# rwl/blu

Hardware: AMD Instinct MI355X
Metric: factorize nnz/s + achieved HBM GB/s, 100k x 100k 10-nnz/col basis (higher is better)
Workload: dtype f64

## Files before the change

### blu_amd/csrc/k_chain.h

```cpp
#pragma once
#include "blu_dev.h"

#define CH_SB 32
#define CH_NB 8
#define CH_CS (CH_SB * CH_NB)
#define CH_CE 4096
#define CH_W 2048
#define CH_FAR 320
#define CH_HAS 0x10000
#define CH_HT 16
#define CH_SEL_FAR (-1)
#define CH_SEL_PREV (-2)

struct __attribute__((aligned(16))) ChRecA {
    int n, eb, w, k;
};
struct __attribute__((aligned(16))) ChRecB {
    double diag, own;
};
struct __attribute__((aligned(16))) ChOpsV {
    double val, xv;
};
struct ChainLds {
    ChOpsV ev[CH_CE];
    int sel[CH_CE];
    double xwin[CH_W];
    ChRecA ra[CH_CS];
    ChRecB rb[CH_CS];
    double rinit[CH_CS];
    long long s_b[CH_CS];
    volatile int blk_ready[CH_NB];
    volatile int eb_tag[CH_HT];
    volatile int eb_val[CH_HT];
    volatile int chain_done;
    volatile int chain_eb;
    volatile int abort;
};

struct ChMeta {
    long long b;
    int len;
    int w;
    double diag, own;
};
struct ChEnt {
    int pos;
    int gidx;
    double val;
};

#define CH_WAIT(L, cond, code)                                         \
    do {                                                            \
        int it_ = 0;                                                \
        while (!(cond)) {                                           \
            if ((L)->abort || ++it_ > (1 << 24)) {                  \
                if (!(L)->abort) (L)->abort = (code);               \
                break;                                              \
            }                                                       \
            __builtin_amdgcn_s_sleep(1);                            \
        }                                                           \
    } while (0)

#ifdef BLU_EMU_BUILD
__device__ __forceinline__ void ch_lds_fence() {}
__device__ __forceinline__ void ch_vm_drain() {}
#else
__device__ __forceinline__ void ch_lds_fence() { asm volatile("s_waitcnt lgkmcnt(0)" ::: "memory"); }
__device__ __forceinline__ void ch_vm_drain() { asm volatile("s_waitcnt vmcnt(0)" ::: "memory"); }
#endif
__device__ __forceinline__ double ch_load_final(gdouble_p p)
{
    const long long b = __hip_atomic_load((GPTR(const long long))p, __ATOMIC_RELAXED, __HIP_MEMORY_SCOPE_AGENT);
    return __longlong_as_double(b);
}

template <bool INIT_OWN, bool SUB, class A>
__device__ __forceinline__ void ch_stage_block(const A &ad, ChainLds *L, int b, int k0, int dir, int nsteps, gdouble_p out)
{
    const int lane = lane_id();
    const int s0 = b * CH_SB;
    const int ns = nsteps - s0 < CH_SB ? nsteps - s0 : CH_SB;
    const int k = k0 + dir * (s0 + (lane < ns ? lane : 0));
    ChMeta M = ad.meta(k);
    if (M.len < 0) M.len = 0;
    const bool mine = lane < ns;
    const int st = (mine && M.len <= 64) ? M.len : 0;
    const int incl = wave_incl_scan_i(st);
    const int off = incl - st;
    const int cnt = __builtin_amdgcn_readlane(incl, 63);
    int base = 0;
    if (b > 0) {
        CH_WAIT(L, L->eb_tag[b & (CH_HT - 1)] == b, 1);
        base = L->eb_val[b & (CH_HT - 1)];
    }
    if (lane == 0) {
        L->eb_val[(b + 1) & (CH_HT - 1)] = base + cnt;
        ch_lds_fence();
        L->eb_tag[(b + 1) & (CH_HT - 1)] = b + 1;
    }
    CH_WAIT(L, L->chain_done >= b - CH_NB + 1 && base + cnt - L->chain_eb <= CH_CE, 2);
    asm volatile("" ::: "memory");
    if (L->abort) return;
    const int slot0 = s0 & (CH_CS - 1);
    if (mine) {
        const int sl = slot0 + lane;
        ChRecA a;
        a.n = M.len <= 64 ? (M.len > 0 ? (M.len | CH_HAS) : 0) : -1;
        a.eb = base + off;
        a.w = M.w;
        a.k = k;
        L->ra[sl] = a;
        ChRecB bq;
        bq.diag = M.diag;
        bq.own = M.own;
        L->rb[sl] = bq;
        L->rinit[sl] = INIT_OWN ? M.own : 0.0;
        L->s_b[sl] = M.b;
    }
    ch_lds_fence();
    for (int f0 = 0; f0 < cnt; f0 += 256) {
        int tt[4], ee[4];
        ChEnt E[4];
        bool ok[4], far[4];
        double xo[4];
#pragma unroll
        for (int u = 0; u < 4; u++) {
            const int f = f0 + u * 64 + lane;
            ok[u] = f < cnt;
            int lo = 0, hi = ns - 1;
            const int target = base + (ok[u] ? f : 0);
#pragma unroll
            for (int it = 0; it < 5; it++) {
                const int mid = (lo + hi + 1) >> 1;
                const bool ge = (L->ra[slot0 + mid].eb <= target) && (mid <= hi);
                lo = ge ? mid : lo;
                hi = ge ? hi : mid - 1;
            }
            tt[u] = lo;
            ee[u] = target - L->ra[slot0 + lo].eb;
        }
#pragma unroll
        for (int u = 0; u < 4; u++) {
            E[u].pos = 0;
            E[u].gidx = 0;
            E[u].val = 0.0;
            if (ok[u]) E[u] = ad.ent(L->ra[slot0 + tt[u]].k, L->s_b[slot0 + tt[u]], ee[u]);
        }
#pragma unroll
        for (int u = 0; u < 4; u++) {
            const int kk = L->ra[slot0 + tt[u]].k;
            const int d = (kk - E[u].pos) * dir;
            far[u] = ok[u] && d >= CH_FAR;
            xo[u] = 0.0;
            if (far[u]) xo[u] = ch_load_final(out + E[u].gidx);
        }
#pragma unroll
        for (int u = 0; u < 4; u++) {
            if (ok[u]) {
                const int kk = L->ra[slot0 + tt[u]].k;
                const int r = (base + f0 + u * 64 + lane) & (CH_CE - 1);
                ChOpsV ov;
                ov.val = E[u].val;
                ov.xv = xo[u];
                L->ev[r] = ov;
                L->sel[r] = far[u] ? CH_SEL_FAR : (E[u].pos == kk - dir ? CH_SEL_PREV : (E[u].pos & (CH_W - 1)));
            }
        }
    }
    ch_lds_fence();
    if (mine && M.len > 0 && M.len <= 64) {
        const int sl = slot0 + lane;
        const int eb = base + off;
        double acc = INIT_OWN ? M.own : 0.0;
        int p = 0;
        while (p < M.len && L->sel[(eb + p) & (CH_CE - 1)] == CH_SEL_FAR) {
            const ChOpsV ov = L->ev[(eb + p) & (CH_CE - 1)];
            const double term = __dmul_rn(ov.xv, ov.val);
            acc = SUB ? __dsub_rn(acc, term) : __dadd_rn(acc, term);
            p++;
        }
        if (p > 0) {
            L->ra[sl].n = (M.len - p) | CH_HAS;
            L->ra[sl].eb = eb + p;
            L->rinit[sl] = acc;
        }
    }
    ch_lds_fence();
    if (lane == 0) L->blk_ready[b & (CH_NB - 1)] = b + 1;
}

struct ChRec {
    int n, eb, w, k;
    double diag, own, init;
};
struct ChOps {
    double val, xv;
    int sel;
};
__device__ __forceinline__ ChRec ch_read_rec(ChainLds *L, int s)
{
    const int sl = s & (CH_CS - 1);
    const ChRecA a = L->ra[sl];
    const ChRecB b = L->rb[sl];
    ChRec R;
    R.n = a.n;
    R.eb = a.eb;
    R.w = a.w;
    R.k = a.k;
    R.diag = b.diag;
    R.own = b.own;
    R.init = L->rinit[sl];
    return R;
}
__device__ __forceinline__ ChOps ch_read_ops(ChainLds *L, const ChRec &R)
{
    ChOps E;
    E.val = 0.0;
    E.xv = 0.0;
    E.sel = CH_SEL_FAR;
    if (lane_id() < (R.n & (CH_HAS - 1)) && R.n > 0) {
        const int r = (R.eb + lane_id()) & (CH_CE - 1);
        const ChOpsV v = L->ev[r];
        E.val = v.val;
        E.xv = v.xv;
        E.sel = L->sel[r];
    }
    return E;
}
template <bool SUB>
__device__ __forceinline__ double ch_accumulate(double acc, double prod, int n)
{
    const unsigned lo = (unsigned)__double_as_longlong(prod), hi = (unsigned)(__double_as_longlong(prod) >> 32);
#define CH_TERM(T)                                                                                              \
    {                                                                                                           \
        const unsigned a_ = __builtin_amdgcn_readlane(lo, (T)), b_ = __builtin_amdgcn_readlane(hi, (T));        \
        const double term_ = __longlong_as_double((long long)(((unsigned long long)b_ << 32) | a_));            \
        acc = SUB ? __dsub_rn(acc, term_) : __dadd_rn(acc, term_);                                              \
    }
    int t = 0;
    for (; t + 4 <= n; t += 4) {
        CH_TERM(t)
        CH_TERM(t + 1)
        CH_TERM(t + 2)
        CH_TERM(t + 3)
    }
    for (; t < n; t++) CH_TERM(t)
#undef CH_TERM
    return acc;
}

template <bool SUB>
__device__ __forceinline__ double ch_accumulate_rows(double acc, double prod, int n)
{
    const double sg = SUB ? -1.0 : 1.0;
#ifdef BLU_EMU_BUILD
#define CH_D(T) acc = fma(__shfl(prod, (lane_id() & ~15) + T), sg, acc);
#define CH_D0 CH_D(0)
#else
#define CH_D(T) asm volatile("v_fmac_f64_dpp %0, %1, %2 row_newbcast:" #T " row_mask:0xf bank_mask:0xf" : "+v"(acc) : "v"(prod), "v"(sg));
#define CH_D0 asm volatile("s_nop 4\n\tv_fmac_f64_dpp %0, %1, %2 row_newbcast:0 row_mask:0xf bank_mask:0xf" : "+v"(acc) : "v"(prod), "v"(sg));
#endif
#define CH_TAIL(A, B, C) \
    if (n > A) {         \
        CH_D(A)          \
        if (n > B) {     \
            CH_D(B)      \
            if (n > C) { \
                CH_D(C)  \
            }            \
        }                \
    }
    if (n >= 4) {
        CH_D0 CH_D(1) CH_D(2) CH_D(3)
        if (n >= 8) {
            CH_D(4) CH_D(5) CH_D(6) CH_D(7)
            if (n >= 12) {
                CH_D(8) CH_D(9) CH_D(10) CH_D(11)
                if (n >= 16) {
                    CH_D(12) CH_D(13) CH_D(14) CH_D(15)
                } else {
                    CH_TAIL(12, 13, 14)
                }
            } else {
                CH_TAIL(8, 9, 10)
            }
        } else {
            CH_TAIL(4, 5, 6)
        }
    } else if (n > 0) {
        CH_D0
        CH_TAIL(1, 2, 3)
    }
#undef CH_TAIL
#undef CH_D0
#undef CH_D
    return acc;
}

template <bool INIT_OWN, bool SUB, class A, class F>
__device__ __forceinline__ bool chain_sweep(const A &ad, ChainLds *L, int k0, int dir, int nsteps, gdouble_p out, F f)
{
    const int w = wave_id(), nw = num_waves(), lane = lane_id();
    const int nblk = (nsteps + CH_SB - 1) / CH_SB;
    if (threadIdx.x < CH_NB) L->blk_ready[threadIdx.x] = 0;
    if (threadIdx.x < CH_HT) L->eb_tag[threadIdx.x] = -1;
    if (threadIdx.x == 0) {
        L->chain_done = 0;
        L->chain_eb = 0;
        L->abort = 0;
    }
    __syncthreads();
    if (w > 0) {
        for (int b = w - 1; b < nblk && !L->abort; b += nw - 1) ch_stage_block<INIT_OWN, SUB>(ad, L, b, k0, dir, nsteps, out);
    } else if (nsteps > 0) {
#ifdef BLU_PROFILE
        long long t_wait = 0, t_drain = 0;
        const long long t_begin = (long long)__builtin_amdgcn_s_memtime();
#endif
        const auto wait_block = [&](int b) {
            if (b < nblk) {
                CH_WAIT(L, L->blk_ready[b & (CH_NB - 1)] == b + 1, 3);
                asm volatile("" ::: "memory");
            }
        };
        const int last = nsteps - 1;
        const auto rl_d = [](double x, int t) {
            const int lo = __builtin_amdgcn_readlane(__double2loint(x), t), hi = __builtin_amdgcn_readlane(__double2hiint(x), t);
            return __hiloint2double(hi, lo);
        };
        const auto read_ops = [&](int eb, int nf) {
            ChOps E;
            E.val = 0.0;
            E.xv = 0.0;
            E.sel = CH_SEL_FAR;
            const int n = nf < 0 ? 0 : (nf & (CH_HAS - 1));
            const int li = n <= 16 ? (lane & 15) : lane;
            if (li < n) {
                const int r = (eb + li) & (CH_CE - 1);
                const ChOpsV v = L->ev[r];
                E.val = v.val;
                E.xv = v.xv;
                E.sel = L->sel[r];
            }
            return E;
        };
        wait_block(0);
        ChRec BR;
        ChOps E1, E2;
        double xw1 = 0.0, vprev = 0.0;
        for (int b = 0; b < nblk && !L->abort; b++) {
#ifdef BLU_PROFILE
            const long long tw0 = (long long)__builtin_amdgcn_s_memtime();
#endif
            wait_block(b + 1);
#ifdef BLU_PROFILE
            t_wait += (long long)__builtin_amdgcn_s_memtime() - tw0;
#endif
            const int bs = b * CH_SB;
            {
                const int sl = bs + lane;
                BR = ch_read_rec(L, sl < last ? sl : last);
            }
            if (b == 0) {
                E1 = read_ops(__builtin_amdgcn_readlane(BR.eb, 0), __builtin_amdgcn_readlane(BR.n, 0));
                xw1 = E1.sel >= 0 ? L->xwin[E1.sel] : 0.0;
                E2 = read_ops(__builtin_amdgcn_readlane(BR.eb, 1), __builtin_amdgcn_readlane(BR.n, 1));
            }
            const int ns = (bs + CH_SB < nsteps ? CH_SB : nsteps - bs);
            for (int t = 0; t < ns; t++) {
                const double xw2 = E2.sel >= 0 ? L->xwin[E2.sel] : 0.0;
                const ChOps E3 = read_ops(__builtin_amdgcn_readlane(BR.eb, t + 2), __builtin_amdgcn_readlane(BR.n, t + 2));
                const int nf = __builtin_amdgcn_readlane(BR.n, t), k1 = __builtin_amdgcn_readlane(BR.k, t), w1 = __builtin_amdgcn_readlane(BR.w, t);
                const double own1 = rl_d(BR.own, t), diag1 = rl_d(BR.diag, t);
                const int n1 = nf < 0 ? -1 : (nf & (CH_HAS - 1));
                double acc = rl_d(BR.init, t);
                if (n1 > 0) {
                    const double x = E1.sel == CH_SEL_PREV ? vprev : (E1.sel >= 0 ? xw1 : E1.xv);
                    if (n1 <= 16) acc = ch_accumulate_rows<SUB>(acc, (lane & 15) < n1 ? __dmul_rn(x, E1.val) : 0.0, n1);
                    else acc = ch_accumulate<SUB>(acc, lane < n1 ? __dmul_rn(x, E1.val) : 0.0, n1);
                } else if (n1 < 0) {
                    const ChMeta M = ad.meta(k1);
                    for (int o = 0; o < M.len; o += 64) {
                        ChEnt E;
                        E.pos = 0;
                        E.gidx = 0;
                        E.val = 0.0;
                        const int nn = M.len - o < 64 ? M.len - o : 64;
                        if (lane < nn) E = ad.ent(k1, M.b, o + lane);
                        acc = ch_accumulate<SUB>(acc, lane < nn ? __dmul_rn(out[E.gidx], E.val) : 0.0, nn);
                    }
                }
                const double v = f(k1, nf != 0, acc, own1, diag1);
                if (lane == 0) {
                    L->xwin[k1 & (CH_W - 1)] = v;
                    out[w1] = v;
                }
                vprev = v;
                E1 = E2;
                xw1 = xw2;
                E2 = E3;
            }
#ifdef BLU_PROFILE
            const long long td0 = (long long)__builtin_amdgcn_s_memtime();
#endif
            ch_vm_drain();
#ifdef BLU_PROFILE
            t_drain += (long long)__builtin_amdgcn_s_memtime() - td0;
#endif
            ch_lds_fence();
            const int eb_next = __builtin_amdgcn_readlane(BR.eb, CH_SB);
            if (lane == 0 && bs + CH_SB < nsteps) {
                L->chain_eb = eb_next;
                L->chain_done = b + 1;
            }
        }
        ch_vm_drain();
#ifdef BLU_PROFILE
        if (lane == 0)
            printf("chain sweep (block %d): %d steps, %.0f cycles/step, waiting for blocks %.0f, draining stores %.0f\n", (int)blockIdx.x, nsteps,
                   (double)((long long)__builtin_amdgcn_s_memtime() - t_begin) / nsteps, (double)t_wait / nsteps, (double)t_drain / nsteps);
#endif
    }
    __syncthreads();
    return L->abort == 0;
}
```

### blu_amd/csrc/k_chain.hip

```cpp
#include "blu_dev.h"
#include "k_chain.h"

struct RowsWs {
    int *lt_ptr, *lt_idx;
    double *lt_val;
    int *lt_cur;
    int *ur_len;
    int *ur_pos;
    double *ur_val;
};

template <bool DESC>
__device__ __forceinline__ void insertion_sort_ik(int *key, double *val, int b, int e)
{
    for (int p = b + 1; p < e; p++) {
        const int k = key[p];
        const double v = val[p];
        int q = p - 1;
        while (q >= b && (DESC ? key[q] < k : key[q] > k)) {
            key[q + 1] = key[q];
            val[q + 1] = val[q];
            q--;
        }
        key[q + 1] = k;
        val[q + 1] = v;
    }
}
template <bool DESC>
__device__ void wave_sort_segment_ik(int *key, double *val, int b, int e, int *lk, double *lv)
{
    const int lane = lane_id();
    const int n = e - b;
    WAVE_LOCKSTEP();
    for (int t = lane; t < n; t += 64) {
        lk[t] = key[b + t];
        lv[t] = val[b + t];
    }
    __builtin_amdgcn_fence(__ATOMIC_SEQ_CST, "workgroup");
    for (int t = lane; t < n; t += 64) {
        const int k = lk[t];
        int r = 0;
        for (int u = 0; u < n; u++) r += DESC ? (lk[u] > k) : (lk[u] < k);
        key[b + r] = k;
        val[b + r] = lv[t];
    }
}

template <class Scope>
__device__ __forceinline__ void rows_body(const DevG &D, const RowsWs &R, Scope &sc, int *lds_k, double *lds_v)
{
    Scalars *S = D.s;
    const int tid = sc.tid(), nt = sc.nt();
    const int m = D.m;
    if (S->status != ST_DONE) return;
    const int rank = S->rank;
    const int lend = D.lbeg[rank];
    for (int i = tid; i < m; i += nt) R.lt_cur[i] = 0;
    if (sc.leader()) *sc.ctr(0) = *sc.ctr(1) = 0;
    sc.sync();
    for (int p = tid; p < lend; p += nt) atomicAdd(&R.lt_cur[D.lidx[p]], 1);
    sc.sync();
    int base = 0;
    for (int c0 = 0; c0 < m; c0 += nt) {
        const int i = c0 + tid;
        const int c = i < m ? R.lt_cur[i] : 0;
        int tot;
        const int ex = sc.excl_scan(c, &tot);
        if (i < m) {
            R.lt_ptr[i] = base + ex;
            R.lt_cur[i] = base + ex;
        }
        base += tot;
    }
    if (sc.leader()) R.lt_ptr[m] = base;
    sc.sync();
    for (int k = tid; k < rank; k += nt)
        for (int p = D.lbeg[k]; p < D.lbeg[k + 1]; p++) {
            const int q = atomicAdd(&R.lt_cur[D.lidx[p]], 1);
            R.lt_idx[q] = k;
            R.lt_val[q] = D.lval[p];
        }
    sc.sync();
    for (int i = tid; i < m; i += nt) {
        const int b = R.lt_ptr[i], e = R.lt_ptr[i + 1];
        if (e - b > 24 && e - b <= WSORT_MAX) D.iw2[atomicAdd(sc.ctr(0), 1)] = i;
        else insertion_sort_ik<false>(R.lt_idx, R.lt_val, b, e);
    }
    for (int k = tid; k < m; k += nt) {
        int n = 0;
        if (k < rank) {
            const int b = D.ubeg[k], e = D.ubeg[k + 1];
            for (int p = b; p < e; p++) {
                const int c = D.qinv[D.uidx[p]];
                if (c < rank) {
                    R.ur_pos[b + n] = c;
                    R.ur_val[b + n] = D.uval[p];
                    n++;
                }
            }
            if (n > 24 && n <= WSORT_MAX) D.iw1[atomicAdd(sc.ctr(1), 1)] = k;
            else insertion_sort_ik<true>(R.ur_pos, R.ur_val, b, b + n);
        }
        R.ur_len[k] = n;
    }
    sc.sync();
    {
        const int nl = __hip_atomic_load(sc.ctr(0), __ATOMIC_RELAXED, __HIP_MEMORY_SCOPE_AGENT);
        const int nu = __hip_atomic_load(sc.ctr(1), __ATOMIC_RELAXED, __HIP_MEMORY_SCOPE_AGENT);
#ifdef BLU_STATS_DEBUG
        if (sc.leader()) printf("k_rows_grid: medium L rows %d, medium U rows %d, rank %d, m %d\n", nl, nu, rank, m);
#endif
        for (int r = sc.wid(); r < nl + nu; r += sc.nw()) {
            if (r < nl) {
                const int i = D.iw2[r];
                wave_sort_segment_ik<false>(R.lt_idx, R.lt_val, R.lt_ptr[i], R.lt_ptr[i + 1], &lds_k[wave_id() * WSORT_MAX],
                                            &lds_v[wave_id() * WSORT_MAX]);
            } else {
                const int k = D.iw1[r - nl];
                wave_sort_segment_ik<true>(R.ur_pos, R.ur_val, D.ubeg[k], D.ubeg[k] + R.ur_len[k], &lds_k[wave_id() * WSORT_MAX],
                                           &lds_v[wave_id() * WSORT_MAX]);
            }
        }
    }
    sc.sync();
    for (int p = tid; p < lend; p += nt) R.lt_idx[p] = D.prow[R.lt_idx[p]];
}
__global__ void __launch_bounds__(1024) k_rows_grid(DevLU *Ds, GridWs *gw, RowsWs R)
{
    __shared__ int sh[40];
    __shared__ long long shl[20];
    __shared__ int lds_k[16 * WSORT_MAX];
    __shared__ double lds_v[16 * WSORT_MAX];
    const DevG D(Ds[0]);
    GridScope sc{sh, shl, gw, 0};
    rows_body(D, R, sc, lds_k, lds_v);
}

struct ChUCols {
    GPTR(const long long) colptr;
    GPTR(const long long) rowidx;
    GPTR(const double) value;
    gdouble_p own;
    __device__ __forceinline__ ChMeta meta(int k) const
    {
        ChMeta M;
        M.b = colptr[k];
        const long long e = colptr[k + 1] - 1;
        M.len = (int)(e - M.b);
        M.w = k;
        M.diag = value[e];
        M.own = own ? ch_load_final(own + k) : 0.0;
        return M;
    }
    __device__ __forceinline__ ChEnt ent(int, long long b, int e) const
    {
        ChEnt E;
        E.pos = (int)rowidx[b + e];
        E.gidx = E.pos;
        E.val = value[b + e];
        return E;
    }
};
struct ChLStage {
    gcint_p lbeg, lidx, pinv;
    gdouble_p lval;
    gdouble_p own;
    __device__ __forceinline__ ChMeta meta(int k) const
    {
        ChMeta M;
        M.b = lbeg[k];
        M.len = lbeg[k + 1] - lbeg[k];
        M.w = k;
        M.diag = 1.0;
        M.own = own ? ch_load_final(own + k) : 0.0;
        return M;
    }
    __device__ __forceinline__ ChEnt ent(int, long long b, int e) const
    {
        ChEnt E;
        E.pos = pinv[lidx[b + e]];
        E.gidx = E.pos;
        E.val = lval[b + e];
        return E;
    }
};
struct ChLRows {
    const int *ptr, *idx;
    const double *v;
    gcint_p prow, pinv;
    gdouble_p own;
    __device__ __forceinline__ ChMeta meta(int k) const
    {
        ChMeta M;
        const int i = prow[k];
        M.b = ptr[i];
        M.len = ptr[i + 1] - ptr[i];
        M.w = k;
        M.diag = 1.0;
        M.own = own ? ch_load_final(own + k) : 0.0;
        return M;
    }
    __device__ __forceinline__ ChEnt ent(int, long long b, int e) const
    {
        ChEnt E;
        E.pos = pinv[idx[b + e]];
        E.gidx = E.pos;
        E.val = v[b + e];
        return E;
    }
};
struct ChURows {
    gcint_p ubeg;
    const int *len, *pos;
    const double *v;
    GPTR(const long long) colptr;
    GPTR(const double) value;
    gdouble_p own;
    __device__ __forceinline__ ChMeta meta(int k) const
    {
        ChMeta M;
        M.b = ubeg[k];
        M.len = len[k];
        M.w = k;
        M.diag = value[colptr[k + 1] - 1];
        M.own = own ? ch_load_final(own + k) : 0.0;
        return M;
    }
    __device__ __forceinline__ ChEnt ent(int, long long b, int e) const
    {
        ChEnt E;
        E.pos = pos[b + e];
        E.gidx = E.pos;
        E.val = v[b + e];
        return E;
    }
};

#define CHAIN_THREADS 512
__global__ void __launch_bounds__(CHAIN_THREADS) k_stats_chains(DevLU *Ds, FinishOut *Os, RowsWs R, int *defect)
{
    BLU_DYN_SHARED(unsigned char, ch_smem, sizeof(ChainLds));
    ChainLds *L = (ChainLds *)ch_smem;
    const DevG D(Ds[0]);
    const FinishOut &O = Os[0];
    Scalars *S = D.s;
    const int m = D.m, lane = lane_id();
    if (S->status != ST_DONE || D.skip_stats) return;
    const size_t M1 = (size_t)(m + 1);
    gdouble_p wl = D.gwork, wu = D.gwork + M1, lf = D.gwork + 2 * M1, rf = D.gwork + 3 * M1, lb = D.gwork + 4 * M1, rb = D.gwork + 5 * M1;
    gdouble_p res = D.gwork + 8 * M1;
    const bool w0 = threadIdx.x < 64;
    const int cc = blockIdx.x;
    bool ok = true;
    if (cc == 0) {
        double x1 = 0.0, xinf = 0.0, y1 = 0.0;
        const ChLStage A1{D.lbeg, D.lidx, D.pinv, D.lval, nullptr};
        ok = ok && chain_sweep<false, false>(A1, L, m - 1, -1, m, wl, [&](int, bool has, double dot, double, double) {
            double temp = has ? -dot : 0.0;
            temp += temp >= 0.0 ? 1.0 : -1.0;
            x1 += fabs(temp);
            xinf = fmax(xinf, fabs(temp));
            return temp;
        });
        const ChLRows A2{R.lt_ptr, R.lt_idx, R.lt_val, D.prow, D.pinv, wl};
        ok = ok && chain_sweep<true, true>(A2, L, 0, 1, m, wl, [&](int, bool, double acc, double, double) {
            y1 += fabs(acc);
            return acc;
        });
        if (w0 && lane == 0) res[0] = fmax(y1 / x1, xinf);
    } else if (cc == 1) {
        double x1 = 0.0, xinf = 0.0, y1 = 0.0;
        const ChUCols A1{(GPTR(const long long))O.u_colptr, (GPTR(const long long))O.u_rowidx, (GPTR(const double))O.u_value, nullptr};
        ok = ok && chain_sweep<false, false>(A1, L, 0, 1, m, wu, [&](int, bool has, double dot, double, double diag) {
            double temp = has ? -dot : 0.0;
            temp += temp >= 0.0 ? 1.0 : -1.0;
            temp /= diag;
            x1 += fabs(temp);
            xinf = fmax(xinf, fabs(temp));
            return temp;
        });
        const ChURows A2{D.ubeg, R.ur_len, R.ur_pos, R.ur_val, (GPTR(const long long))O.u_colptr, (GPTR(const double))O.u_value, wu};
        ok = ok && chain_sweep<true, true>(A2, L, m - 1, -1, m, wu, [&](int, bool, double acc, double, double diag) {
            const double temp = acc / diag;
            y1 += fabs(temp);
            return temp;
        });
        if (w0 && lane == 0) res[1] = fmax(y1 / x1, xinf);
    } else if (cc == 2) {
        const ChLRows A1{R.lt_ptr, R.lt_idx, R.lt_val, D.prow, D.pinv, nullptr};
        ok = ok && chain_sweep<false, false>(A1, L, 0, 1, m, lf, [&](int k, bool, double d, double, double) {
            const double r = d <= 0.0 ? 1.0 : -1.0;
            if (lane == 0) rf[k] = r;
            return r - d;
        });
        const ChURows A2{D.ubeg, R.ur_len, R.ur_pos, R.ur_val, (GPTR(const long long))O.u_colptr, (GPTR(const double))O.u_value, lf};
        ok = ok && chain_sweep<true, true>(A2, L, m - 1, -1, m, lf, [&](int, bool, double acc, double, double diag) { return acc / diag; });
    } else {
        const ChUCols A1{(GPTR(const long long))O.u_colptr, (GPTR(const long long))O.u_rowidx, (GPTR(const double))O.u_value, nullptr};
        ok = ok && chain_sweep<false, false>(A1, L, 0, 1, m, lb, [&](int k, bool has, double dot, double, double diag) {
            const double d = has ? dot : 0.0;
            const double r = d <= 0.0 ? 1.0 : -1.0;
            if (lane == 0) rb[k] = r;
            return (r - d) / diag;
        });
        const ChLStage A2{D.lbeg, D.lidx, D.pinv, D.lval, lb};
        ok = ok && chain_sweep<false, false>(A2, L, m - 1, -1, m, lb, [&](int, bool has, double dot, double own, double) { return has ? own - dot : own; });
    }
    if (!ok && threadIdx.x == 0) atomicMax(defect, L->abort ? L->abort : 99);
}

#define TAIL_BLOCKS 64
__global__ void __launch_bounds__(1024) k_stats_tail_a(DevLU *Ds, FinishOut *Os, GridWs *gw)
{
    const DevG D(Ds[0]);
    const FinishOut &O = Os[0];
    Scalars *S = D.s;
    __shared__ double red[4][40];
    if (S->status != ST_DONE || D.skip_stats) return;
    double v[4];
    stats_tail_loops<false>(D, O, (int)(blockIdx.x * blockDim.x + threadIdx.x), (int)(gridDim.x * blockDim.x), v[0], v[1], v[2], v[3],
                            &gw->nlong);
    for (int q = 0; q < 4; q++) {
        const double x = wave_max_d(v[q]);
        if (lane_id() == 0) red[q][wave_id()] = x;
    }
    __syncthreads();
    if (threadIdx.x < 4) {
        double a = red[threadIdx.x][0];
        for (int ww = 1; ww < num_waves(); ww++) a = fmax(a, red[threadIdx.x][ww]);
        ((double *)gw->partll[0])[4 * blockIdx.x + threadIdx.x] = a;
    }
}
__global__ void __launch_bounds__(1024) k_stats_tail_b(DevLU *Ds, FinishOut *Os, GridWs *gw)
{
    const DevG D(Ds[0]);
    Scalars *S = D.s;
    __shared__ double red[4][40];
    __shared__ double chain_out[16];
    if (S->status != ST_DONE || D.skip_stats) return;
    const size_t M1 = (size_t)(D.m + 1);
    if (threadIdx.x < 2) chain_out[threadIdx.x] = D.gwork[8 * M1 + threadIdx.x];
    double v[4] = {0.0, 0.0, 0.0, 0.0};
    if (threadIdx.x < TAIL_BLOCKS)
        for (int q = 0; q < 4; q++) v[q] = ((const double *)gw->partll[0])[4 * threadIdx.x + q];
    const int nlong = gw->nlong;
    if (nlong && wave_id() < 4)
        v[3] = fmax(v[3], stats_long_rows(D.bt_ptr, D.bt_idx, D.bt_val, D.qinv, D.pinv, D.gwork, D.m, S->rank, nlong, wave_id(), 4));
    __syncthreads();
    stats_tail_finish(D, red, chain_out, v[0], v[1], v[2], v[3]);
    const size_t ng = 7 * M1;
    for (size_t e = threadIdx.x; e < ng; e += blockDim.x) D.gwork[e] = 0.0;
    if (threadIdx.x < 2) D.gwork[8 * M1 + threadIdx.x] = 0.0;
}

struct ChSolveLRows {
    const int *ptr, *idx;
    const double *v;
    gcint_p prow, pinv;
    gdouble_p y;
    __device__ __forceinline__ ChMeta meta(int k) const
    {
        ChMeta M;
        const int i = prow[k];
        M.b = ptr[i];
        M.len = ptr[i + 1] - ptr[i];
        M.w = i;
        M.diag = 1.0;
        M.own = ch_load_final(y + i);
        return M;
    }
    __device__ __forceinline__ ChEnt ent(int, long long b, int e) const
    {
        ChEnt E;
        E.gidx = idx[b + e];
        E.pos = pinv[E.gidx];
        E.val = v[b + e];
        return E;
    }
};
struct ChSolveURows {
    gcint_p ubeg;
    const int *len, *pos;
    const double *v;
    GPTR(const long long) colptr;
    GPTR(const double) value;
    gcint_p prow, pcol;
    gdouble_p y;
    __device__ __forceinline__ ChMeta meta(int k) const
    {
        ChMeta M;
        M.b = ubeg[k];
        M.len = len[k];
        M.w = pcol[k];
        M.diag = value[colptr[k + 1] - 1];
        M.own = ch_load_final(y + prow[k]);
        return M;
    }
    __device__ __forceinline__ ChEnt ent(int, long long b, int e) const
    {
        ChEnt E;
        E.pos = pos[b + e];
        E.gidx = pcol[E.pos];
        E.val = v[b + e];
        return E;
    }
};
struct ChSolveUCols {
    GPTR(const long long) colptr;
    GPTR(const long long) rowidx;
    GPTR(const double) value;
    gcint_p prow, pcol;
    gdouble_p y;
    __device__ __forceinline__ ChMeta meta(int k) const
    {
        ChMeta M;
        M.b = colptr[k];
        const long long e = colptr[k + 1] - 1;
        M.len = (int)(e - M.b);
        M.w = prow[k];
        M.diag = value[e];
        M.own = ch_load_final(y + pcol[k]);
        return M;
    }
    __device__ __forceinline__ ChEnt ent(int, long long b, int e) const
    {
        ChEnt E;
        E.pos = (int)rowidx[b + e];
        E.gidx = prow[E.pos];
        E.val = value[b + e];
        return E;
    }
};
struct ChSolveLStage {
    gcint_p lbeg, lidx, pinv, prow;
    gdouble_p lval;
    gdouble_p x;
    __device__ __forceinline__ ChMeta meta(int k) const
    {
        ChMeta M;
        M.b = lbeg[k];
        M.len = lbeg[k + 1] - lbeg[k];
        M.w = prow[k];
        M.diag = 1.0;
        M.own = ch_load_final(x + M.w);
        return M;
    }
    __device__ __forceinline__ ChEnt ent(int, long long b, int e) const
    {
        ChEnt E;
        E.gidx = lidx[b + e];
        E.pos = pinv[E.gidx];
        E.val = lval[b + e];
        return E;
    }
};

__global__ void __launch_bounds__(CHAIN_THREADS) k_solve_dense_chain(DevLU *Ds, FinishOut *Os, RowsWs R, const double *rhs, double *lhs, int trans,
                                                                     int *defect)
{
    BLU_DYN_SHARED(unsigned char, ch_smem, sizeof(ChainLds));
    ChainLds *L = (ChainLds *)ch_smem;
    const DevG D(Ds[0]);
    const FinishOut &O = Os[0];
    const int m = D.m;
    gdouble_p y = D.txrj;
    gdouble_p x_out = (gdouble_p)lhs;
    for (int k = threadIdx.x; k < m; k += blockDim.x) y[k] = rhs[k];
    ch_vm_drain();
    __syncthreads();
    const auto sub_dot = [](int, bool has, double dot, double own, double) { return has ? own - dot : own; };
    const auto over_diag = [](int, bool, double acc, double, double diag) { return acc / diag; };
    bool ok = true;
    if (!trans) {
        const ChSolveLRows A1{R.lt_ptr, R.lt_idx, R.lt_val, D.prow, D.pinv, y};
        ok = ok && chain_sweep<false, false>(A1, L, 0, 1, m, y, sub_dot);
        const ChSolveURows A2{D.ubeg, R.ur_len, R.ur_pos, R.ur_val, (GPTR(const long long))O.u_colptr, (GPTR(const double))O.u_value, D.prow, D.pcol, y};
        ok = ok && chain_sweep<true, true>(A2, L, m - 1, -1, m, x_out, over_diag);
    } else {
        const ChSolveUCols A1{(GPTR(const long long))O.u_colptr, (GPTR(const long long))O.u_rowidx, (GPTR(const double))O.u_value, D.prow, D.pcol, y};
        ok = ok && chain_sweep<true, true>(A1, L, 0, 1, m, x_out, over_diag);
        const ChSolveLStage A2{D.lbeg, D.lidx, D.pinv, D.prow, D.lval, x_out};
        ok = ok && chain_sweep<false, false>(A2, L, m - 1, -1, m, x_out, sub_dot);
    }
    if (threadIdx.x == 0) *defect = ok ? 0 : 9100 + L->abort;
}
```

Measured before the change: 1.313 million.

## Finish fully-far chain steps in helper waves and stage refined diagonal reciprocals

Helper (staging) waves now compute the final value of any step whose operands all come from far, already-final entries, and mark it CH_FIN. The serial wave then writes whole runs of finished steps in one batch instead of walking through them one by one. Helpers also stage a refined reciprocal of each diagonal, so the serial path can replace full f64 division with a div_scale/fma/fixup sequence when no scaling is needed. The value callback is split into a value part and a fold part so helper waves can evaluate it. This adds LDS footprint and branch complexity, and the reciprocal fast path has to match IEEE division exactly.

```diff
diff --git a/blu_amd/csrc/k_chain.h b/blu_amd/csrc/k_chain.h
--- a/blu_amd/csrc/k_chain.h
+++ b/blu_amd/csrc/k_chain.h
@@ -1,4 +1,5 @@
 #pragma once
+#include <type_traits>
 #include "blu_dev.h"
 
 #define CH_SB 32
@@ -8,6 +9,7 @@
 #define CH_W 2048
 #define CH_FAR 320
 #define CH_HAS 0x10000
+#define CH_FIN 0x20000
 #define CH_HT 16
 #define CH_SEL_FAR (-1)
 #define CH_SEL_PREV (-2)
@@ -17,6 +19,10 @@
 };
 struct __attribute__((aligned(16))) ChRecB {
     double diag, own;
+};
+struct __attribute__((aligned(16))) ChRecC {
+    double init;
+    double rdiag;
 };
 struct __attribute__((aligned(16))) ChOpsV {
     double val, xv;
@@ -27,7 +33,7 @@
     double xwin[CH_W];
     ChRecA ra[CH_CS];
     ChRecB rb[CH_CS];
-    double rinit[CH_CS];
+    ChRecC rc[CH_CS];
     long long s_b[CH_CS];
     volatile int blk_ready[CH_NB];
     volatile int eb_tag[CH_HT];
@@ -35,6 +41,10 @@
     volatile int chain_done;
     volatile int chain_eb;
     volatile int abort;
+#ifdef BLU_STATS_DEBUG
+    int dbg_div[2];
+    int dbg_fin[2];
+#endif
 };
 
 struct ChMeta {
@@ -74,8 +84,43 @@
     return __longlong_as_double(b);
 }
 
-template <bool INIT_OWN, bool SUB, class A>
-__device__ __forceinline__ void ch_stage_block(const A &ad, ChainLds *L, int b, int k0, int dir, int nsteps, gdouble_p out)
+__device__ __forceinline__ double ch_rcp_refined(double y)
+{
+#ifdef BLU_EMU_BUILD
+    return 1.0 / y;
+#else
+    const double r0 = __builtin_amdgcn_rcp(y);
+    const double e0 = __builtin_fma(-y, r0, 1.0);
+    const double r1 = __builtin_fma(r0, e0, r0);
+    const double e1 = __builtin_fma(-y, r1, 1.0);
+    return __builtin_fma(r1, e1, r1);
+#endif
+}
+__device__ __forceinline__ void ch_dbg_div(ChainLds *L, bool full)
+{
+#ifdef BLU_STATS_DEBUG
+    if (lane_id() == 0) L->dbg_div[full ? 1 : 0]++;
+#endif
+}
+__device__ __forceinline__ double ch_div(double x, double y, double r, ChainLds *L)
+{
+#ifndef BLU_EMU_BUILD
+    bool fy, fx;
+    const double ys = __builtin_amdgcn_div_scale(x, y, false, &fy);
+    const double xs = __builtin_amdgcn_div_scale(x, y, true, &fx);
+    if (__double_as_longlong(ys) == __double_as_longlong(y) && __double_as_longlong(xs) == __double_as_longlong(x) && !fx) {
+        ch_dbg_div(L, false);
+        const double q = __dmul_rn(xs, r);
+        const double t = __builtin_fma(-ys, q, xs);
+        return __builtin_amdgcn_div_fixup(__builtin_amdgcn_div_fmas(t, r, q, fx), y, x);
+    }
+#endif
+    ch_dbg_div(L, true);
+    return x / y;
+}
+
+template <bool INIT_OWN, bool SUB, class A, class V>
+__device__ __forceinline__ void ch_stage_block(const A &ad, ChainLds *L, int b, int k0, int dir, int nsteps, gdouble_p out, V val)
 {
     const int lane = lane_id();
     const int s0 = b * CH_SB;
@@ -114,7 +159,6 @@
         bq.diag = M.diag;
         bq.own = M.own;
         L->rb[sl] = bq;
-        L->rinit[sl] = INIT_OWN ? M.own : 0.0;
         L->s_b[sl] = M.b;
     }
     ch_lds_fence();
@@ -168,22 +212,29 @@
         }
     }
     ch_lds_fence();
-    if (mine && M.len > 0 && M.len <= 64) {
+    if (mine) {
         const int sl = slot0 + lane;
         const int eb = base + off;
-        double acc = INIT_OWN ? M.own : 0.0;
-        int p = 0;
-        while (p < M.len && L->sel[(eb + p) & (CH_CE - 1)] == CH_SEL_FAR) {
-            const ChOpsV ov = L->ev[(eb + p) & (CH_CE - 1)];
-            const double term = __dmul_rn(ov.xv, ov.val);
-            acc = SUB ? __dsub_rn(acc, term) : __dadd_rn(acc, term);
-            p++;
-        }
-        if (p > 0) {
-            L->ra[sl].n = (M.len - p) | CH_HAS;
-            L->ra[sl].eb = eb + p;
-            L->rinit[sl] = acc;
-        }
+        ChRecC c;
+        c.init = INIT_OWN ? M.own : 0.0;
+        c.rdiag = ch_rcp_refined(M.diag);
+        if (M.len <= 64) {
+            int p = 0;
+            while (p < M.len && L->sel[(eb + p) & (CH_CE - 1)] == CH_SEL_FAR) {
+                const ChOpsV ov = L->ev[(eb + p) & (CH_CE - 1)];
+                const double term = __dmul_rn(ov.xv, ov.val);
+                c.init = SUB ? __dsub_rn(c.init, term) : __dadd_rn(c.init, term);
+                p++;
+            }
+            if (p == M.len) {
+                c.init = val(false, k, M.len > 0, c.init, M.own, M.diag, c.rdiag);
+                L->ra[sl].n = CH_FIN;
+            } else if (p > 0) {
+                L->ra[sl].n = (M.len - p) | CH_HAS;
+                L->ra[sl].eb = eb + p;
+            }
+        }
+        L->rc[sl] = c;
     }
     ch_lds_fence();
     if (lane == 0) L->blk_ready[b & (CH_NB - 1)] = b + 1;
@@ -191,7 +242,7 @@
 
 struct ChRec {
     int n, eb, w, k;
-    double diag, own, init;
+    double diag, own, init, rdiag;
 };
 struct ChOps {
     double val, xv;
@@ -209,7 +260,9 @@
     R.k = a.k;
     R.diag = b.diag;
     R.own = b.own;
-    R.init = L->rinit[sl];
+    const ChRecC c = L->rc[sl];
+    R.init = c.init;
+    R.rdiag = c.rdiag;
     return R;
 }
 __device__ __forceinline__ ChOps ch_read_ops(ChainLds *L, const ChRec &R)
@@ -297,8 +350,11 @@
     return acc;
 }
 
-template <bool INIT_OWN, bool SUB, class A, class F>
-__device__ __forceinline__ bool chain_sweep(const A &ad, ChainLds *L, int k0, int dir, int nsteps, gdouble_p out, F f)
+struct ChNoFold {
+    __device__ __forceinline__ void operator()(double) const {}
+};
+template <bool INIT_OWN, bool SUB, class A, class V, class G>
+__device__ __forceinline__ bool chain_sweep(const A &ad, ChainLds *L, int k0, int dir, int nsteps, gdouble_p out, V val, G fold)
 {
     const int w = wave_id(), nw = num_waves(), lane = lane_id();
     const int nblk = (nsteps + CH_SB - 1) / CH_SB;
@@ -308,13 +364,17 @@
         L->chain_done = 0;
         L->chain_eb = 0;
         L->abort = 0;
+#ifdef BLU_STATS_DEBUG
+        L->dbg_div[0] = L->dbg_div[1] = L->dbg_fin[0] = L->dbg_fin[1] = 0;
+#endif
     }
     __syncthreads();
     if (w > 0) {
-        for (int b = w - 1; b < nblk && !L->abort; b += nw - 1) ch_stage_block<INIT_OWN, SUB>(ad, L, b, k0, dir, nsteps, out);
+        for (int b = w - 1; b < nblk && !L->abort; b += nw - 1) ch_stage_block<INIT_OWN, SUB>(ad, L, b, k0, dir, nsteps, out, val);
     } else if (nsteps > 0) {
 #ifdef BLU_PROFILE
-        long long t_wait = 0, t_drain = 0;
+        long long t_wait = 0, t_drain = 0, t_fin = 0;
+        int n_fin = 0, n_run = 0;
         const long long t_begin = (long long)__builtin_amdgcn_s_memtime();
 #endif
         const auto wait_block = [&](int b) {
@@ -367,11 +427,47 @@
                 E2 = read_ops(__builtin_amdgcn_readlane(BR.eb, 1), __builtin_amdgcn_readlane(BR.n, 1));
             }
             const int ns = (bs + CH_SB < nsteps ? CH_SB : nsteps - bs);
-            for (int t = 0; t < ns; t++) {
+            const unsigned long long finm = __ballot(lane < ns && BR.n > 0 && (BR.n & CH_FIN) != 0);
+            for (int t = 0; t < ns;) {
+                if ((finm >> t) & 1) {
+#ifdef BLU_PROFILE
+                    const long long tf0 = (long long)__builtin_amdgcn_s_memtime();
+#endif
+                    const int r = __ffsll((long long)~(finm >> t)) - 1;
+                    const int e = t + r;
+                    const ChOps N1 = r == 1 ? E2 : read_ops(__builtin_amdgcn_readlane(BR.eb, e), __builtin_amdgcn_readlane(BR.n, e));
+                    double xwn = 0.0;
+                    if (r == 1) xwn = N1.sel >= 0 ? L->xwin[N1.sel] : 0.0;
+                    const ChOps N2 = read_ops(__builtin_amdgcn_readlane(BR.eb, e + 1), __builtin_amdgcn_readlane(BR.n, e + 1));
+                    if (lane >= t && lane < e) {
+                        L->xwin[BR.k & (CH_W - 1)] = BR.init;
+                        out[BR.w] = BR.init;
+                    }
+                    if constexpr (!std::is_same<G, ChNoFold>::value)
+                        for (int u = t; u < e; u++) fold(rl_d(BR.init, u));
+                    vprev = rl_d(BR.init, e - 1);
+                    E1 = N1;
+                    E2 = N2;
+                    if (r > 1) xwn = E1.sel >= 0 ? L->xwin[E1.sel] : 0.0;
+                    xw1 = xwn;
+                    t = e;
+#ifdef BLU_PROFILE
+                    t_fin += (long long)__builtin_amdgcn_s_memtime() - tf0;
+                    n_fin += r;
+                    n_run++;
+#endif
+#ifdef BLU_STATS_DEBUG
+                    if (lane == 0) {
+                        L->dbg_fin[0] += r;
+                        L->dbg_fin[1]++;
+                    }
+#endif
+                    continue;
+                }
                 const double xw2 = E2.sel >= 0 ? L->xwin[E2.sel] : 0.0;
                 const ChOps E3 = read_ops(__builtin_amdgcn_readlane(BR.eb, t + 2), __builtin_amdgcn_readlane(BR.n, t + 2));
                 const int nf = __builtin_amdgcn_readlane(BR.n, t), k1 = __builtin_amdgcn_readlane(BR.k, t), w1 = __builtin_amdgcn_readlane(BR.w, t);
-                const double own1 = rl_d(BR.own, t), diag1 = rl_d(BR.diag, t);
+                const double own1 = rl_d(BR.own, t), diag1 = rl_d(BR.diag, t), rd1 = rl_d(BR.rdiag, t);
                 const int n1 = nf < 0 ? -1 : (nf & (CH_HAS - 1));
                 double acc = rl_d(BR.init, t);
                 if (n1 > 0) {
@@ -390,7 +486,8 @@
                         acc = ch_accumulate<SUB>(acc, lane < nn ? __dmul_rn(out[E.gidx], E.val) : 0.0, nn);
                     }
                 }
-                const double v = f(k1, nf != 0, acc, own1, diag1);
+                const double v = val(true, k1, nf != 0, acc, own1, diag1, rd1);
+                fold(v);
                 if (lane == 0) {
                     L->xwin[k1 & (CH_W - 1)] = v;
                     out[w1] = v;
@@ -399,6 +496,7 @@
                 E1 = E2;
                 xw1 = xw2;
                 E2 = E3;
+                t++;
             }
 #ifdef BLU_PROFILE
             const long long td0 = (long long)__builtin_amdgcn_s_memtime();
@@ -417,8 +515,14 @@
         ch_vm_drain();
 #ifdef BLU_PROFILE
         if (lane == 0)
-            printf("chain sweep (block %d): %d steps, %.0f cycles/step, waiting for blocks %.0f, draining stores %.0f\n", (int)blockIdx.x, nsteps,
-                   (double)((long long)__builtin_amdgcn_s_memtime() - t_begin) / nsteps, (double)t_wait / nsteps, (double)t_drain / nsteps);
+            printf("chain sweep (block %d): %d steps, %.0f cycles/step, waiting for blocks %.0f, draining stores %.0f; finished by helpers %d in %d runs, "
+                   "%.0f cycles each\n", (int)blockIdx.x, nsteps, (double)((long long)__builtin_amdgcn_s_memtime() - t_begin) / nsteps,
+                   (double)t_wait / nsteps, (double)t_drain / nsteps, n_fin, n_run, n_fin ? (double)t_fin / n_fin : 0.0);
+#endif
+#ifdef BLU_STATS_DEBUG
+        if (lane == 0)
+            printf("chain sweep (block %d): %d steps, finished by helpers %d in %d runs, divisions by the staged reciprocal %d, in full %d\n",
+                   (int)blockIdx.x, nsteps, L->dbg_fin[0], L->dbg_fin[1], L->dbg_div[0], L->dbg_div[1]);
 #endif
     }
     __syncthreads();
diff --git a/blu_amd/csrc/k_chain.hip b/blu_amd/csrc/k_chain.hip
--- a/blu_amd/csrc/k_chain.hip
+++ b/blu_amd/csrc/k_chain.hip
@@ -252,59 +252,60 @@
     const bool w0 = threadIdx.x < 64;
     const int cc = blockIdx.x;
     bool ok = true;
+    const auto over_diag = [&](bool chain, int, bool, double acc, double, double diag, double rdiag) {
+        return chain ? ch_div(acc, diag, rdiag, L) : acc / diag;
+    };
     if (cc == 0) {
         double x1 = 0.0, xinf = 0.0, y1 = 0.0;
         const ChLStage A1{D.lbeg, D.lidx, D.pinv, D.lval, nullptr};
-        ok = ok && chain_sweep<false, false>(A1, L, m - 1, -1, m, wl, [&](int, bool has, double dot, double, double) {
+        const auto fold_x = [&](double temp) {
+            x1 += fabs(temp);
+            xinf = fmax(xinf, fabs(temp));
+        };
+        ok = ok && chain_sweep<false, false>(A1, L, m - 1, -1, m, wl, [](bool, int, bool has, double dot, double, double, double) {
             double temp = has ? -dot : 0.0;
             temp += temp >= 0.0 ? 1.0 : -1.0;
-            x1 += fabs(temp);
-            xinf = fmax(xinf, fabs(temp));
             return temp;
-        });
+        }, fold_x);
         const ChLRows A2{R.lt_ptr, R.lt_idx, R.lt_val, D.prow, D.pinv, wl};
-        ok = ok && chain_sweep<true, true>(A2, L, 0, 1, m, wl, [&](int, bool, double acc, double, double) {
-            y1 += fabs(acc);
-            return acc;
-        });
+        ok = ok && chain_sweep<true, true>(A2, L, 0, 1, m, wl, [](bool, int, bool, double acc, double, double, double) { return acc; },
+                                           [&](double v) { y1 += fabs(v); });
         if (w0 && lane == 0) res[0] = fmax(y1 / x1, xinf);
     } else if (cc == 1) {
         double x1 = 0.0, xinf = 0.0, y1 = 0.0;
         const ChUCols A1{(GPTR(const long long))O.u_colptr, (GPTR(const long long))O.u_rowidx, (GPTR(const double))O.u_value, nullptr};
-        ok = ok && chain_sweep<false, false>(A1, L, 0, 1, m, wu, [&](int, bool has, double dot, double, double diag) {
+        const auto fold_x = [&](double temp) {
+            x1 += fabs(temp);
+            xinf = fmax(xinf, fabs(temp));
+        };
+        ok = ok && chain_sweep<false, false>(A1, L, 0, 1, m, wu, [&](bool chain, int, bool has, double dot, double, double diag, double rdiag) {
             double temp = has ? -dot : 0.0;
             temp += temp >= 0.0 ? 1.0 : -1.0;
-            temp /= diag;
-            x1 += fabs(temp);
-            xinf = fmax(xinf, fabs(temp));
-            return temp;
-        });
+            return chain ? ch_div(temp, diag, rdiag, L) : temp / diag;
+        }, fold_x);
         const ChURows A2{D.ubeg, R.ur_len, R.ur_pos, R.ur_val, (GPTR(const long long))O.u_colptr, (GPTR(const double))O.u_value, wu};
-        ok = ok && chain_sweep<true, true>(A2, L, m - 1, -1, m, wu, [&](int, bool, double acc, double, double diag) {
-            const double temp = acc / diag;
-            y1 += fabs(temp);
-            return temp;
-        });
+        ok = ok && chain_sweep<true, true>(A2, L, m - 1, -1, m, wu, over_diag, [&](double v) { y1 += fabs(v); });
         if (w0 && lane == 0) res[1] = fmax(y1 / x1, xinf);
     } else if (cc == 2) {
         const ChLRows A1{R.lt_ptr, R.lt_idx, R.lt_val, D.prow, D.pinv, nullptr};
-        ok = ok && chain_sweep<false, false>(A1, L, 0, 1, m, lf, [&](int k, bool, double d, double, double) {
+        ok = ok && chain_sweep<false, false>(A1, L, 0, 1, m, lf, [&](bool chain, int k, bool, double d, double, double, double) {
             const double r = d <= 0.0 ? 1.0 : -1.0;
-            if (lane == 0) rf[k] = r;
+            if (!chain || lane == 0) rf[k] = r;
             return r - d;
-        });
+        }, ChNoFold());
         const ChURows A2{D.ubeg, R.ur_len, R.ur_pos, R.ur_val, (GPTR(const long long))O.u_colptr, (GPTR(const double))O.u_value, lf};
-        ok = ok && chain_sweep<true, true>(A2, L, m - 1, -1, m, lf, [&](int, bool, double acc, double, double diag) { return acc / diag; });
+        ok = ok && chain_sweep<true, true>(A2, L, m - 1, -1, m, lf, over_diag, ChNoFold());
     } else {
         const ChUCols A1{(GPTR(const long long))O.u_colptr, (GPTR(const long long))O.u_rowidx, (GPTR(const double))O.u_value, nullptr};
-        ok = ok && chain_sweep<false, false>(A1, L, 0, 1, m, lb, [&](int k, bool has, double dot, double, double diag) {
+        ok = ok && chain_sweep<false, false>(A1, L, 0, 1, m, lb, [&](bool chain, int k, bool has, double dot, double, double diag, double rdiag) {
             const double d = has ? dot : 0.0;
             const double r = d <= 0.0 ? 1.0 : -1.0;
-            if (lane == 0) rb[k] = r;
-            return (r - d) / diag;
-        });
+            if (!chain || lane == 0) rb[k] = r;
+            return chain ? ch_div(r - d, diag, rdiag, L) : (r - d) / diag;
+        }, ChNoFold());
         const ChLStage A2{D.lbeg, D.lidx, D.pinv, D.lval, lb};
-        ok = ok && chain_sweep<false, false>(A2, L, m - 1, -1, m, lb, [&](int, bool has, double dot, double own, double) { return has ? own - dot : own; });
+        ok = ok && chain_sweep<false, false>(A2, L, m - 1, -1, m, lb,
+                                             [](bool, int, bool has, double dot, double own, double, double) { return has ? own - dot : own; }, ChNoFold());
     }
     if (!ok && threadIdx.x == 0) atomicMax(defect, L->abort ? L->abort : 99);
 }
@@ -468,19 +469,21 @@
     for (int k = threadIdx.x; k < m; k += blockDim.x) y[k] = rhs[k];
     ch_vm_drain();
     __syncthreads();
-    const auto sub_dot = [](int, bool has, double dot, double own, double) { return has ? own - dot : own; };
-    const auto over_diag = [](int, bool, double acc, double, double diag) { return acc / diag; };
+    const auto sub_dot = [](bool, int, bool has, double dot, double own, double, double) { return has ? own - dot : own; };
+    const auto over_diag = [&](bool chain, int, bool, double acc, double, double diag, double rdiag) {
+        return chain ? ch_div(acc, diag, rdiag, L) : acc / diag;
+    };
     bool ok = true;
     if (!trans) {
         const ChSolveLRows A1{R.lt_ptr, R.lt_idx, R.lt_val, D.prow, D.pinv, y};
-        ok = ok && chain_sweep<false, false>(A1, L, 0, 1, m, y, sub_dot);
+        ok = ok && chain_sweep<false, false>(A1, L, 0, 1, m, y, sub_dot, ChNoFold());
         const ChSolveURows A2{D.ubeg, R.ur_len, R.ur_pos, R.ur_val, (GPTR(const long long))O.u_colptr, (GPTR(const double))O.u_value, D.prow, D.pcol, y};
-        ok = ok && chain_sweep<true, true>(A2, L, m - 1, -1, m, x_out, over_diag);
+        ok = ok && chain_sweep<true, true>(A2, L, m - 1, -1, m, x_out, over_diag, ChNoFold());
     } else {
         const ChSolveUCols A1{(GPTR(const long long))O.u_colptr, (GPTR(const long long))O.u_rowidx, (GPTR(const double))O.u_value, D.prow, D.pcol, y};
-        ok = ok && chain_sweep<true, true>(A1, L, 0, 1, m, x_out, over_diag);
+        ok = ok && chain_sweep<true, true>(A1, L, 0, 1, m, x_out, over_diag, ChNoFold());
         const ChSolveLStage A2{D.lbeg, D.lidx, D.pinv, D.prow, D.lval, x_out};
-        ok = ok && chain_sweep<false, false>(A2, L, m - 1, -1, m, x_out, sub_dot);
+        ok = ok && chain_sweep<false, false>(A2, L, m - 1, -1, m, x_out, sub_dot, ChNoFold());
     }
     if (threadIdx.x == 0) *defect = ok ? 0 : 9100 + L->abort;
 }
```

Result: no change. 1.302 million (-0.8%).
